# cortes-ciriano-lab/DeMethify

Hardware: AMD Instinct MI355X
Metric: NMF update iters/sec (1e6 CpG x 256 samples x 16 types) (higher is better)
Workload: dtype f64; 1 GPU; headline_1e6x256_12+4; N_cpg=1000000, S_samples=256, n_known=12, n_unknown=4, inner_iters=20, restarts=64, restart_seed=1 + k, restart_placement=k mod n_gpus, parallelism=restart-sharded x1

## Files before the change

### demethify_amd/csrc/dmf_api.h

```cpp
#pragma once
#include <hip/hip_runtime.h>

#include <cmath>
#include <cstdio>
#include <cstdlib>
#include <cstring>
#include <memory>
#include <mutex>
#include <new>
#include <unordered_map>
#include <utility>
#include <vector>

#include "../../include/demethify_hip.h"
#include "dmf_internal.h"
#include "dmf_select.h"

using dmf::SolverState;

namespace dmf_api {

int hip_fail(hipError_t e, const char* what, const char* file, int line);

#define HIP_TRY(expr)                                                                          \
// ... 146 lines not shown
    int64_t N16 = 0, plane_stride = 0;
    dmf_api::DevBuf<unsigned short> X16;
    double x16_dev = 0.0, x16_sum = 0.0;
    bool d_f32_exact = false;
    dmf_api::DevBuf<double> gb_known;
    dmf::GramRan known_ran;
    dmf_api::DevBuf<unsigned char> mask_bits;
    dmf_api::DevBuf<unsigned short> W16;
    int64_t n_test = 0;
    dmf::ProblemView view() const {
        dmf::ProblemView v;
        v.V = V, v.D = D, v.D16 = D16, v.X16 = X16, v.Dt8 = Dt8;
        v.plane_stride = plane_stride, v.SD = SD, v.ND = ND;
        v.Rt = Rt, v.Rtp = Rtp;
        v.N = N, v.S = (int)S, v.n_c = (int)n_c;
        return v;
    }
};

constexpr size_t kPinnedStateBytes = (sizeof(SolverState) + 15) / 16 * 16 + 16;

struct dmf_solver {
    dmf_context* ctx = nullptr;
    const dmf_problem* p = nullptr;
    int64_t n_u = 0;
    int mode = 0;
    dmf::ShapeKey key;
    dmf::PathSpec spec;
    dmf_api::DevBuf<double> cm;
    dmf_api::DevBuf<double> beta_tab;
    int64_t beta_cap = 0;
    dmf_api::DevBuf<long long> slab_i8;
    int64_t slab_i8_words = 0;
    dmf_api::DevBuf<long long> acc_i8;
    dmf_api::DevBuf<double> purity;
    dmf_api::DevBuf<double> u2_partials;
    dmf_api::DevBuf<double> u, u_prev, u_next;
    dmf_api::DevBuf<double> alpha, alpha_prev;
    dmf_api::DevBuf<double> gb;
    dmf::GramRan last_gram;
    int last_gram_source = -1;
    dmf_api::DevBuf<double> slab;
    int64_t slab_doubles = 0;
    dmf_api::DevBuf<double> partials;
    dmf_api::DevBuf<SolverState> state;
    SolverState* h_state = nullptr;
    dmf_api::JobTable jobs;
    bool cf_pending = true;
    double* mom_host = nullptr;
    dmf_api::DevBuf<double> mom_dev;
    hipEvent_t cost_event = nullptr;
    bool cost_pending = false;
    bool in_flight = false;
    bool confirm_stops = false;
    double cf_stream = 0.0;
    long long cf_stream_iter = -1;
    long long n_rowpass = 0, n_rowpass_pair = 0;
    long long n_confirmed = 0, n_unconfirmed = 0;
    dmf::IterateView iterate() const {
        dmf::IterateView it;
        it.u = u, it.u_prev = u_prev, it.alpha = alpha, it.state = state;
        it.n_u = (int)n_u, it.mode = mode;
        return it;
    }
    dmf::AlphaView alpha_view() const {
        dmf::AlphaView a;
        a.gb = gb, a.alpha = alpha, a.alpha_prev = alpha_prev, a.purity = purity, a.state = state, a.partials = partials;
// ... 78 lines not shown
```

### demethify_amd/csrc/dmf_api_problem.hip

```cpp
#include "dmf_api.h"

namespace dmf_api {

static int alloc_count_copies(dmf_problem* p, int ND, bool x16, bool w16) {
    dmf_context* ctx = p->ctx;
    p->ND = ND;
    p->SD = (int)((p->S + 63) / 64 * 64);
    p->N16 = (p->N + 15) / 16 * 16;
    p->plane_stride = ((p->N + 31) / 32) * (p->SD / 32) * 1024;
    const size_t u16_elems = (size_t)p->N16 * p->SD;
    HIP_TRY(p->D16.alloc(ctx, u16_elems));
    HIP_TRY(p->Dt8.alloc(ctx, (size_t)p->plane_stride * ND));
    if (x16) HIP_TRY(p->X16.alloc(ctx, u16_elems));
    if (w16) HIP_TRY(p->W16.alloc(ctx, u16_elems));
    return DMF_OK;
}

static void known_route(dmf_problem* p, const char* piece) {
    char* t = p->known_ran.text;
    const size_t have = std::strlen(t), cap = sizeof(p->known_ran.text);
    snprintf(t + have, cap - have, "%s%s", have > 0 ? " " : "", piece);
}

static int problem_finalize(dmf_problem* p, bool counts_done = false) {
// ... 45 lines not shown
                p->X16.reset();
            } else {
                std::memcpy(&p->x16_dev, &got[1], sizeof(double));
                p->x16_sum = (double)got[2];
            }
        }
    }

    if (n_c > 0 && n_c <= 48) {
        const int nct = (int)((n_c + 3) / 4 * 4);
        if (nct == n_c) {
            p->Rtp.borrow(p->Rt);
        } else {
            HIP_TRY(p->Rtp.alloc(ctx, (size_t)N * nct));
            HIP_TRY(dmf::launch_pad_rows(p->Rt, p->Rtp, N, (int)n_c, nct, ctx->stream));
        }
    }

    const dmf::ProblemView pv = p->view();
    JobTable jobs;
    jobs.build(0, (int)n_c, [](int, int) { return true; });
    const int n_jobs = jobs.n;
    const bool mfma = n_c >= 1 && ctx->generic_level != 1 && ctx->generic_level != 2;
    const int n_fast = mfma ? n_jobs - 1 : 0, n_dense = (int)(n_c * (n_c + 1) / 2);
    const bool int_known = mfma && ctx->generic_level == 0 && p->Dt8 != nullptr && p->D16 != nullptr && p->Rtp != nullptr &&
                           (reinterpret_cast<uintptr_t>(p->Rtp.get()) & 15) == 0 &&
                           dmf::gram_i8_known_supported((int)n_c, p->ND, N, p->SD);
    int64_t slab_doubles = dmf::gram_slab_doubles(N, (int)S, mfma ? 1 : n_jobs);
    if (mfma && !int_known) {
        const int64_t need = dmf::gram_mfma_slab_doubles(N, (int)S, n_fast);
        if (need > slab_doubles) slab_doubles = need;
    }
    DevBuf<double> slab, slab_bu;
    DevBuf<long long> slab_i8, acc;
    HIP_TRY(p->gb_known.alloc(ctx, (size_t)n_jobs * S));
    DMF_TRY(jobs.upload(ctx));
    HIP_TRY(slab.alloc(ctx, (size_t)slab_doubles));
    bool vdv_done = true;
    if (int_known) {
        const int64_t slab_words = dmf::gram_i8_slab_words_nf(N, p->SD, n_dense);
        const int64_t acc_words = dmf::gram_i8_acc_words_nf((int)S, n_dense, (int)n_c + 1);
        HIP_TRY(slab_i8.alloc(ctx, (size_t)slab_words));
        HIP_TRY(acc.alloc(ctx, (size_t)acc_words));
        HIP_TRY(slab_bu.alloc(ctx, (size_t)dmf::bu_cols_grid(N) * (n_c + 1) * S));
        HIP_TRY(hipMemsetAsync(acc, 0, (size_t)acc_words * sizeof(long long), ctx->stream));
        int ny = 0, n_slabs = 0;
        dmf::GramRan ran;
        HIP_TRY(dmf::launch_gram_i8(pv, nullptr, 0, jobs.k, jobs.l, n_dense, slab_i8, slab_words, nullptr, &ny, ctx->stream, &ran));
        known_route(p, "int_known");
        known_route(p, ran.text);
        HIP_TRY(dmf::launch_bu_cols(pv, p->Rt, (int)n_c, slab_bu, nullptr, &n_slabs, ctx->stream, &vdv_done));
        known_route(p, vdv_done ? "+ k_bu_cols2 with vDv" : "+ k_bu_cols");
        HIP_TRY(dmf::launch_gram_v2_reduce(slab_i8, ny, n_dense, p->SD, slab_bu, n_slabs, (int)n_c + (vdv_done ? 1 : 0), (int)S,
                                           acc, jobs.dst, p->gb_known, nullptr, nullptr, 0, nullptr, ctx->stream));
    } else if (mfma) {
        dmf::GramJobTable fast{jobs.k, jobs.l, jobs.dst, n_fast};
        int ny = 0;
        dmf::GramRan ran;
        HIP_TRY(dmf::launch_gram_mfma(pv, nullptr, 0, fast, n_dense, slab, slab_doubles, nullptr, &ny, ctx->stream, &ran));
        known_route(p, "fp64");
        known_route(p, ran.text);
        HIP_TRY(dmf::launch_gram_reduce(slab, ny, n_fast, (int)S, jobs.dst, p->gb_known, nullptr, ctx->stream));
    }
    if (int_known && vdv_done) {
    } else if (n_jobs - n_fast == 1 && ctx->generic_level != 1 && ctx->generic_level != 2 &&
               (int64_t)dmf::vdv_cols_grid(N) * S <= slab_doubles) {
        HIP_TRY(dmf::launch_vdv_cols(pv, slab, p->gb_known + (int64_t)jobs.h_dst[n_jobs - 1] * S, ctx->stream));
        known_route(p, p->known_ran.text[0] == 0 ? "fp64 k_vdv_cols" : "+ k_vdv_cols");
    } else {
        dmf::GramJobTable rest{jobs.k + n_fast, jobs.l + n_fast, jobs.dst + n_fast, n_jobs - n_fast};
        dmf::GramRan ran;
        if (p->known_ran.text[0] == 0) known_route(p, "fp64");
        else known_route(p, "+");
        HIP_TRY(dmf::launch_gram(pv, nullptr, 0, rest, slab, slab_doubles, p->gb_known, nullptr, ctx->stream, &ran));
        known_route(p, ran.text);
    }
    HIP_TRY(hipStreamSynchronize(ctx->stream));
    return DMF_OK;
}

static dmf::CostPlan cost_plan_of(dmf_context* ctx, const dmf::ProblemView& p, int n_u) {
    return dmf::cost_plan(dmf::cost_key(p, n_u, ctx->generic_level));
}

hipError_t enqueue_cost(dmf_context* ctx, const dmf::ProblemView& p, const double* u, const double* alpha, int n_u,
                        double* scratch, double* out) {
    return dmf::launch_cost_plan(cost_plan_of(ctx, p, n_u), p, u, alpha, n_u, scratch, out, ctx->stream);
// ... 251 lines not shown
```

### demethify_amd/csrc/dmf_api_solver.hip

```cpp
#include "dmf_api.h"

namespace dmf_api {

using dmf::kSplitInnerSteps;

static int ensure_split_scratch(dmf_solver* s, int n_iter2) {
    dmf_context* ctx = s->ctx;
    if (s->cm == nullptr) HIP_TRY(s->cm.alloc(ctx, (size_t)dmf::u_phase_split_cm_doubles(s->p->N, (int)s->n_u)));
    if (s->beta_cap < n_iter2 || s->beta_tab == nullptr) {
        s->beta_cap = n_iter2 > 0 ? n_iter2 : 1;
        HIP_TRY(s->beta_tab.alloc(ctx, (size_t)s->beta_cap));
    }
    return DMF_OK;
}

int enqueue_u_phase(dmf_solver* s, int n_iter2, dmf::RowKind row) {
    dmf_context* ctx = s->ctx;
    const dmf::ProblemView pv = s->p->view();
    FamilyScope scope(ctx, DMF_KERNEL_ROWPASS);
    switch (row) {
        case dmf::RowKind::CmI8InnerRows:
            DMF_TRY(ensure_split_scratch(s, n_iter2));
            HIP_TRY(dmf::launch_u_phase_split_i8(pv, s->iterate(), n_iter2, s->scratch(), ctx->stream));
            return DMF_OK;
        case dmf::RowKind::UPhaseBig:
            HIP_TRY(dmf::launch_u_phase_big(pv, s->iterate(), n_iter2, ctx->stream));
            return DMF_OK;
        case dmf::RowKind::UPhaseMfmaSplit:
            DMF_TRY(ensure_split_scratch(s, n_iter2));
            HIP_TRY(dmf::launch_u_phase_split(pv, s->iterate(), n_iter2, s->scratch(), ctx->stream));
            return DMF_OK;
        case dmf::RowKind::UPhaseMfma:
            HIP_TRY(dmf::launch_u_phase_mfma(pv, s->iterate(), n_iter2, ctx->stream));
            return DMF_OK;
        case dmf::RowKind::UPhaseGram:
            HIP_TRY(dmf::launch_u_phase_gram(pv, s->iterate(), n_iter2, ctx->stream));
            return DMF_OK;
        case dmf::RowKind::UStepDirect:
            for (int t = 0; t < n_iter2; ++t) {
                HIP_TRY(dmf::launch_u_step_direct(pv, s->iterate(), s->u_next, t, ctx->stream));
                std::swap(s->u_prev, s->u);
                std::swap(s->u, s->u_next);
            }
            return DMF_OK;
        default: return DMF_ERR_BAD_ARG;
    }
}

dmf::RowKind standalone_row_kind(const dmf_solver* s, int n_iter2) {
    return dmf::plan_iteration(s->key, dmf::standalone_spec(s->spec), n_iter2, false).row;
}

struct GramI8Buffers {
    double* slab_bu = nullptr;
    long long* slab_i8 = nullptr;
    int64_t slab_i8_words = 0;
    long long* acc = nullptr;
    double* gb = nullptr;
    const int* done = nullptr;
};

static GramI8Buffers solver_i8_buffers(dmf_solver* s) {
    GramI8Buffers b;
    b.slab_bu = s->slab, b.slab_i8 = s->slab_i8, b.slab_i8_words = s->slab_i8_words, b.acc = s->acc_i8, b.gb = s->gb;
    b.done = &s->state->done;
    return b;
}

static int gram_i8_and_reduce(dmf_solver* s, const GramI8Buffers& b, int n_slabs, const double* u2_partials, int n_u2,
                              dmf::GramRan* ran = nullptr) {
    dmf_context* ctx = s->ctx;
    const dmf_problem* p = s->p;
    const int S = (int)p->S, n_c = (int)p->n_c, n_u = (int)s->n_u, nf = n_c * n_u + n_u * (n_u + 1) / 2;
    int ny = 0;
    HIP_TRY(dmf::launch_gram_i8(p->view(), s->u, n_u, s->jobs.k, s->jobs.l, nf, b.slab_i8, b.slab_i8_words, b.done, &ny,
                                ctx->stream, ran));
    HIP_TRY(dmf::launch_gram_v2_reduce(b.slab_i8, ny, nf, p->SD, b.slab_bu, n_slabs, n_u, S, b.acc, s->jobs.dst, b.gb, b.done,
                                       u2_partials, n_u2, s->state, ctx->stream));
    return DMF_OK;
}

static int gram_bu_cols_i8(dmf_solver* s, const GramI8Buffers& b, dmf::GramRan* ran = nullptr) {
    int n_slabs = 0;
    HIP_TRY(dmf::launch_bu_cols(s->p->view(), s->u, (int)s->n_u, b.slab_bu, b.done, &n_slabs, s->ctx->stream));
    return gram_i8_and_reduce(s, b, n_slabs, nullptr, 0, ran);
}

int enqueue_gram(dmf_solver* s, dmf::GramKind kind, bool heed_done, dmf::GramRan* ran) {
    dmf_context* ctx = s->ctx;
    const dmf::ProblemView pv = s->p->view();
    const int S = pv.S, n_u = (int)s->n_u;
    const int* done = heed_done ? &s->state->done : nullptr;
    FamilyScope scope(ctx, DMF_KERNEL_GRAM);
    if (kind == dmf::GramKind::BuColsI8) {
        GramI8Buffers b = solver_i8_buffers(s);
        b.done = done;
        return gram_bu_cols_i8(s, b, ran);
    }
    if (kind == dmf::GramKind::GramU) {
        int ny = 0;
        HIP_TRY(dmf::launch_gram_u(pv, s->u, n_u, s->slab, done, &ny, ctx->stream, ran));
        HIP_TRY(dmf::launch_gram_reduce(s->slab, ny, s->jobs.n, S, s->jobs.dst, s->gb, done, ctx->stream));
        return DMF_OK;
    }
    dmf::GramJobTable jobs{s->jobs.k, s->jobs.l, s->jobs.dst, s->jobs.n};
    if (kind == dmf::GramKind::GramMfma) {
        int ny = 0;
        HIP_TRY(dmf::launch_gram_mfma(pv, s->u, n_u, jobs, s->jobs.n - n_u, s->slab, s->slab_doubles, done, &ny, ctx->stream, ran));
        HIP_TRY(dmf::launch_gram_reduce(s->slab, ny, s->jobs.n, S, s->jobs.dst, s->gb, done, ctx->stream));
        return DMF_OK;
    }
// ... 222 lines not shown
    if (s->spec.use_fused) {
        const int64_t spec = dmf::rowpass_fused_slab_doubles(N - (N & 15), (int)S, (int)n_c, (int)n_u) +
                             dmf::gram_u_slab_doubles(16, (int)S, (int)n_c, (int)n_u);
        if (spec > s->slab_doubles) s->slab_doubles = spec;
    }
    if (s->spec.use_v2) {
        const int64_t bu = (int64_t)dmf::rowpass_v2_grid(N, (int)S) * n_u * S;
        if (bu > s->slab_doubles) s->slab_doubles = bu;
    }
    if (s->spec.use_gram_i8) {
        const int64_t bu = (int64_t)dmf::bu_cols_grid(N) * n_u * S;
        if (bu > s->slab_doubles) s->slab_doubles = bu;
        if (s->spec.use_cm_i8) {
            const int64_t bu2 = (int64_t)dmf::u_inner_bu_grid(N, (int)S) * n_u * S;
            if (bu2 > s->slab_doubles) s->slab_doubles = bu2;
        }
    }
    const size_t un = (size_t)N * n_u, an = (size_t)K * S;
    const size_t un_alloc = (un + 1) & ~(size_t)1;
    const size_t gbn = (size_t)(K + 1) * (K + 2) / 2 * S;
    const int nb_alpha = (int)((S + 63) / 64);
    HIP_TRY(s->u.alloc(ctx, un_alloc));
    HIP_TRY(s->u_prev.alloc(ctx, un_alloc));
    if (s->spec.u_path == 2) HIP_TRY(s->u_next.alloc(ctx, un_alloc));
    HIP_TRY(s->alpha.alloc(ctx, an));
    HIP_TRY(s->alpha_prev.alloc(ctx, an));
    HIP_TRY(s->gb.alloc(ctx, gbn));
    HIP_TRY(s->slab.alloc(ctx, (size_t)s->slab_doubles));
    HIP_TRY(s->partials.alloc(ctx, (size_t)2 * (nb_alpha + S)));
    HIP_TRY(s->u2_partials.alloc(ctx, 4096));
    if (s->spec.use_v2 || s->spec.use_gram_i8) {
        s->slab_i8_words = dmf::gram_i8_slab_words(N, p->SD, (int)n_c, (int)n_u);
        HIP_TRY(s->slab_i8.alloc(ctx, (size_t)s->slab_i8_words));
        const size_t acc_words = (size_t)dmf::gram_i8_acc_words((int)S, (int)n_c, (int)n_u);
        HIP_TRY(s->acc_i8.alloc(ctx, acc_words));
        HIP_TRY(hipMemsetAsync(s->acc_i8, 0, acc_words * sizeof(long long), ctx->stream));
    }
    HIP_TRY(s->state.alloc(ctx, 1));
    if (!ctx->pinned_states.empty()) {
        s->h_state = (SolverState*)ctx->pinned_states.back();
        ctx->pinned_states.pop_back();
    } else {
        HIP_TRY(hipHostMalloc((void**)&s->h_state, kPinnedStateBytes));
    }
    const hipMemcpyKind in_kind = (flags & DMF_PTR_DEVICE) ? hipMemcpyDeviceToDevice : hipMemcpyHostToDevice;
    HIP_TRY(hipMemsetAsync(s->state, 0, sizeof(SolverState), ctx->stream));
    HIP_TRY(hipMemsetAsync(s->gb, 0, gbn * sizeof(double), ctx->stream));
    HIP_TRY(hipMemcpyAsync(s->u, u0, un * sizeof(double), in_kind, ctx->stream));
    HIP_TRY(hipMemcpyAsync(s->u_prev, s->u, un * sizeof(double), hipMemcpyDeviceToDevice, ctx->stream));
    HIP_TRY(hipMemcpyAsync(s->alpha, alpha0, an * sizeof(double), in_kind, ctx->stream));
    HIP_TRY(hipMemcpyAsync(s->alpha_prev, s->alpha, an * sizeof(double), hipMemcpyDeviceToDevice, ctx->stream));
    DMF_TRY(s->jobs.upload(ctx));
    HIP_TRY(dmf::launch_scatter_known_block(p->gb_known, s->gb, (int)n_c, (int)K, (int)S, ctx->stream));
    HIP_TRY(dmf::launch_sumsq_f64(s->u, N * n_u, ctx->scratch, &s->state->u_norm2, nullptr, ctx->stream));
    HIP_TRY(dmf::launch_init_state(s->state, p->consts, s->alpha, (int)S, (int)n_c, (int)n_u, ctx->stream));
    if (!(flags & DMF_PTR_DEVICE)) HIP_TRY(hipStreamSynchronize(ctx->stream));
    return DMF_OK;
}

}

using namespace dmf_api;

extern "C" {

int dmf_solver_create(dmf_context* ctx, const dmf_problem* p, const double* u0, const double* alpha0,
                      int64_t n_u, int mode, int flags, dmf_solver** out) {
    DMF_TRY(check_ctx(ctx));
    if (out == nullptr) return DMF_ERR_BAD_ARG;
// ... 140 lines not shown
    *out_cost = *cost_slot(s);
    return DMF_OK;
}

int dmf_solver_holdout_error(dmf_solver* s, const dmf_problem* full, double* sum_sq, int64_t* n_test) {
    if (s == nullptr || full == nullptr || sum_sq == nullptr || n_test == nullptr) return DMF_ERR_BAD_ARG;
    dmf_context* ctx = s->ctx;
    DMF_TRY(check_ctx(ctx));
    const dmf_problem* p = s->p;
    if (p->mask_bits == nullptr || full->mask_bits != nullptr || full->ctx != ctx) return DMF_ERR_BAD_ARG;
    if (full->N != p->N || full->S != p->S || full->n_c != p->n_c) return DMF_ERR_BAD_SHAPE;
    *n_test = p->n_test;
    *sum_sq = 0.0;
    if (p->n_test == 0) return DMF_OK;
    dmf::ProblemView pv;
    pv.N = p->N, pv.S = (int)p->S, pv.n_c = (int)p->n_c;
    pv.V = full->V, pv.Rt = p->Rt, pv.Rtp = p->Rtp;
    pv.D16 = p->W16, pv.SD = p->SD;
    DevBuf<double> weights;
    if (!cost_reads_u16_only(ctx, pv, (int)s->n_u)) {
        HIP_TRY(weights.alloc(ctx, (size_t)p->N * p->S));
        HIP_TRY(dmf::launch_holdout_weights_f64(p->mask_bits, weights, p->N, (int)p->S, ctx->stream));
        pv.D = weights, pv.D16 = nullptr, pv.SD = 0;
    }
    return cost_to_host(ctx, pv, s->u, s->alpha, (int)s->n_u, sum_sq, true);
}

static int solver_gram_enqueue(dmf_solver* s, int kind, double* out_gb, dmf::GramRan* ran) {
    dmf_context* ctx = s->ctx;
    const dmf_problem* p = s->p;
    const int64_t N = p->N, S = p->S, n_c = p->n_c, n_u = s->n_u, K = n_c + n_u;
    const size_t gbn = (size_t)(K + 1) * (K + 2) / 2 * S;
    DevBuf<double> slab_bu;
    DevBuf<long long> slab_i8, acc;
    if (kind == DMF_GRAM_LAST) {
        *ran = s->last_gram;
    } else if (kind == DMF_GRAM_FP64) {
        DMF_TRY(enqueue_gram(s, fp64_gram_kind(s), false, ran));
    } else {
        GramI8Buffers b;
        b.slab_i8_words = dmf::gram_i8_slab_words(N, p->SD, (int)n_c, (int)n_u);
        const size_t acc_words = (size_t)dmf::gram_i8_acc_words((int)S, (int)n_c, (int)n_u);
        HIP_TRY(slab_bu.alloc(ctx, (size_t)dmf::bu_cols_grid(N) * n_u * S));
        HIP_TRY(slab_i8.alloc(ctx, (size_t)b.slab_i8_words));
        HIP_TRY(acc.alloc(ctx, acc_words));
        HIP_TRY(hipMemsetAsync(acc, 0, acc_words * sizeof(long long), ctx->stream));
        b.slab_bu = slab_bu, b.slab_i8 = slab_i8, b.acc = acc, b.gb = s->gb;
        FamilyScope scope(ctx, DMF_KERNEL_GRAM);
        DMF_TRY(gram_bu_cols_i8(s, b, ran));
    }
    HIP_TRY(hipMemcpyAsync(out_gb, s->gb, gbn * sizeof(double), hipMemcpyDeviceToHost, ctx->stream));
    HIP_TRY(hipStreamSynchronize(ctx->stream));
    return DMF_OK;
}

int dmf_solver_gram(dmf_solver* s, int kind, double* out_gb, char* out_text, int64_t cap) {
    if (s == nullptr || out_gb == nullptr || (kind != DMF_GRAM_INTEGER && kind != DMF_GRAM_FP64 && kind != DMF_GRAM_LAST))
        return DMF_ERR_BAD_ARG;
    if (out_text != nullptr && cap < 1) return DMF_ERR_BAD_ARG;
    dmf_context* ctx = s->ctx;
    DMF_TRY(check_ctx(ctx));
    const dmf_problem* p = s->p;
    if (kind == DMF_GRAM_INTEGER &&
        (p->ND < 1 || p->D16 == nullptr || p->Dt8 == nullptr || (p->n_c > 0 && p->Rtp == nullptr) ||
         (reinterpret_cast<uintptr_t>(p->Rtp.get()) & 15) != 0 ||
         !dmf::gram_i8_supported((int)p->n_c, (int)s->n_u, p->ND, p->N, p->SD)))
        return DMF_ERR_UNSUPPORTED;
    dmf::GramRan ran;
    s->in_flight = true;
    const int status = solver_gram_enqueue(s, kind, out_gb, &ran);
    if (status != DMF_OK) (void)hipStreamSynchronize(ctx->stream);
    s->in_flight = false;
    if (status == DMF_OK && out_text != nullptr) snprintf(out_text, (size_t)cap, "%s", ran.text);
    return status;
}

static dmf::RowKind row_moments_kind(const dmf_solver* s) { return standalone_row_kind(s, kSplitInnerSteps + 1); }

static int solver_row_moments_enqueue(dmf_solver* s, dmf::RowKind row, double* out_cm, dmf::CmRan* ran) {
    dmf_context* ctx = s->ctx;
// ... 114 lines not shown
```

### demethify_amd/csrc/dmf_internal.h

```cpp
#pragma once
#include <hip/hip_runtime.h>
#include <stdint.h>

#include "dmf_select.h"

namespace dmf {

struct SolverState {
    double a1;
    double a2;
    double l_w;
    double l_w_prev;
    double l_h;
    double l_h_prev;
    double dsq;
    double rt_norm2;
    double u_norm2;
    double cf;
    double cf_prev;
    double tol;
    long long iters;
    double band;
    int done;
    int arrive;
// ... 246 lines not shown
constexpr double kX16MaxDev = 8.0 * 0x1p-53;
hipError_t launch_build_counts_int(const double* D, const double* V, int64_t N, int S, int ND, unsigned short* D16,
                                   unsigned short* X16, int64_t N16, int SD, signed char* Dt8, int64_t plane_stride,
                                   unsigned long long* x_stats, hipStream_t st);
hipError_t launch_build_dt8(const unsigned short* D16, int64_t N, int SD, int ND, signed char* Dt8, int64_t plane_stride,
                            hipStream_t st);
hipError_t launch_mask_problem(const double* srcV, const double* srcD, const unsigned short* src16,
                               const unsigned short* srcX, const unsigned char* bits, double* dstV, double* dstD,
                               unsigned short* dst16, unsigned short* dstX, unsigned short* W16, int64_t N, int64_t N16, int S,
                               int SD, unsigned long long* stats, hipStream_t st);
hipError_t launch_holdout_weights_f64(const unsigned char* bits, double* W, int64_t N, int S, hipStream_t st);
constexpr int64_t kMaskDrawMaxS = ((int64_t)1 << 31) - 1, kMaskDrawMaxElements = (int64_t)1 << 60;
hipError_t launch_mask_draw(unsigned int* key_io, int pos, int64_t N, int64_t S, unsigned long long threshold,
                            unsigned char* bits, unsigned long long* result, hipStream_t st);
bool rowpass_v2_supported(int S, int n_c, int n_u, int n_iter2);
int rowpass_v2_grid(int64_t N, int S);
hipError_t launch_rowpass_v2(const ProblemView& p, const IterateView& it, int n_iter2, const UScratch& scratch, int* grid_out,
                             bool pair, bool* paired_out, hipStream_t st);
bool rowpass_v2_pair_fits(int S, int n_u, int n_iter2);
bool gram_i8_supported(int n_c, int n_u, int ND, int64_t N, int SD);
struct GramI8Plan {
    bool supported = false;
    int xl = 1, nd = 1, ring = 8;
    int nf = 0, launches = 0;
    int nsh = 0, ny = 0;
    int64_t rows_per_wg = 0;
    int blocks = 0, last = 0;
    int tail = 0;
    bool xcd = false;
};
GramI8Plan gram_i8_plan(int64_t N, int SD, int n_c, int n_u, int ND);
void describe_gram_i8_plan(const GramI8Plan& g, char* buf, size_t cap);
int64_t gram_i8_slab_words(int64_t N, int SD, int n_c, int n_u);
int64_t gram_i8_acc_words(int S, int n_c, int n_u);
bool gram_i8_known_supported(int n_c, int ND, int64_t N, int SD);
int64_t gram_i8_slab_words_nf(int64_t N, int SD, int nf);
int64_t gram_i8_acc_words_nf(int S, int nf, int n_bu);
hipError_t launch_gram_i8(const ProblemView& p, const double* u, int n_u, const short* feat_a, const short* feat_b, int NF,
                          long long* slab, int64_t slab_words, const int* done_flag, int* ny_out, hipStream_t st,
                          GramRan* ran = nullptr);
int bu_cols_grid(int64_t N);
hipError_t launch_bu_cols(const ProblemView& p, const double* u, int n_u, double* slab, const int* done_flag,
                          int* n_slabs_out, hipStream_t st, bool* with_vdv = nullptr);
hipError_t launch_gram_v2_reduce(const long long* slab_i8, int ny, int NF, int SD, const double* slab_bu, int n_bu_slabs,
                                 int n_u, int S, long long* acc_words, const int* dst_row, double* gb, const int* done_flag,
                                 const double* u2_partials, int n_u2, SolverState* state, hipStream_t st);

hipError_t launch_percentile_pair(const double* x, int64_t n, int64_t m, PercentilePlan p0, PercentilePlan p1,
                                  double* out0, double* out1, hipStream_t st);
hipError_t launch_nanpercentile_pair(const double* x, int64_t n, int64_t m, PercentilePlan p0, PercentilePlan p1, double q0,
                                     double q1, double* out0, double* out1, hipStream_t st);
int64_t percentile_max_replicates();

int wls_moments_grid(int64_t N);
int64_t wls_slab_doubles(int64_t N, int S, int K);
hipError_t launch_wls_moments(const ProblemView& p, const double* u, int n_u, int target_dv, double* slab, double* mom,
                              hipStream_t st);
hipError_t launch_nnls_intercept(const double* gb, const double* mom, int K, int S, double* out, int* status, hipStream_t st);

constexpr int kSvdMaxS = 512, kSvdMaxNc = 64, kSvdMaxRank = 64;
constexpr size_t kSvdMaxLds = 160 * 1024;
size_t svd_project_lds_bytes(int S, int rank);
struct SvdColumns {
    double sign[kSvdMaxRank], scale[kSvdMaxRank];
};
bool svd_supported(int S, int n_c, int rank);
int svd_gram_grid(int64_t N, int S);
int64_t svd_gram_slab_doubles(int64_t N, int S);
hipError_t launch_svd_gram(const ProblemView& p, const double* H1, double* slab, int* flags, double* C, hipStream_t st);
int64_t svd_project_slab_doubles(int64_t N, int rank);
hipError_t launch_svd_project(const ProblemView& p, const double* H1, const double* Es, int rank, double* T, double* slab,
                              double* norms, hipStream_t st);
hipError_t launch_svd_finish(double* T, int64_t N, int rank, const SvdColumns& cols, hipStream_t st);

struct MatchColumns {
    int src[kMaxK];
};
int match_gram_grid(int64_t N, int n_u);
// ... 13 lines not shown
```

### demethify_amd/csrc/dmf_kernels_gram_i8.hip

```cpp
#include <cstdint>
#include <cstdio>
#include <cstdlib>

#include "dmf_device.h"
#include "dmf_dispatch.h"
#include "dmf_internal.h"
#include "dmf_fixedpoint.h"

namespace dmf {

typedef int v4i __attribute__((ext_vector_type(4)));
typedef int v16i __attribute__((ext_vector_type(16)));
typedef unsigned int v4u __attribute__((ext_vector_type(4)));

namespace {
constexpr int kNSL = 7;
constexpr int kRing = 8;
constexpr int kMaxFeat = 576;
}

__global__ __launch_bounds__(256) void k_build_d16(const double* __restrict__ D, const double* __restrict__ V, int64_t N, int S,
                                                   unsigned short* __restrict__ D16, unsigned short* __restrict__ X16,
                                                   int64_t N16, int SD, unsigned long long* __restrict__ x_stats) {
    const int64_t chunks = N16 * (SD / 8);
// ... 588 lines not shown
    }
}

int bu_cols_grid(int64_t N) {
    int64_t want = (N + 4 * 8 - 1) / (4 * 8);
    if (want > 512) want = 512;
    return (int)(want < 1 ? 1 : want);
}

hipError_t launch_bu_cols(const ProblemView& p, const double* u, int n_u, double* slab, const int* done_flag,
                          int* n_slabs_out, hipStream_t st, bool* with_vdv) {
    const int S = p.S, nbx = bu_cols_grid(p.N);
    *n_slabs_out = nbx;
    const dim3 block(256);
    const bool two = (p.SD & 1) == 0 && S >= 128 && n_u <= 16 && (p.v_align() & 7) == 0;
    const int vdv = (with_vdv != nullptr && *with_vdv && two) ? 1 : 0;
    if (with_vdv != nullptr) *with_vdv = vdv != 0;
    if (two && n_u >= 1) {
        const dim3 grid2(nbx, (S + 127) / 128);
        return dispatch_int<1, 16>(n_u, [&](auto nu) {
            hipLaunchKernelGGL((k_bu_cols2<decltype(nu)::value>), grid2, block, 0, st, p.V, p.D16, p.SD, u, p.N, S, slab,
                               done_flag, vdv);
            return hipGetLastError();
        });
    }
    const dim3 grid(nbx, (S + 63) / 64);
    return dispatch_int<1, 32>(n_u, [&](auto nu) {
        hipLaunchKernelGGL((k_bu_cols<decltype(nu)::value>), grid, block, 0, st, p.V, p.D16, p.SD, u, p.N, S, slab, done_flag);
        return hipGetLastError();
    });
}

constexpr int kRedChunks = 16;

__global__ __launch_bounds__(256) void k_gram_v2_reduce(const long long* __restrict__ slab_i8, int ny, int MF, int SDs,
                                                        const double* __restrict__ slab_bu, int n_bu_slabs, int n_u,
                                                        int n_feat, int S, unsigned long long* __restrict__ acc64,
                                                        double* __restrict__ bu_part,
                                                        const int* __restrict__ done_flag,
                                                        const double* __restrict__ u2_partials, int n_u2,
                                                        SolverState* __restrict__ state) {
    __shared__ long long part[3][2][64];
    __shared__ double partd[3][64];
    if (done_flag != nullptr && *done_flag) return;
    const int lane = threadIdx.x & 63, grp = threadIdx.x >> 6;
    const int s = blockIdx.x * 64 + lane;
    const int job = blockIdx.y, chunk = blockIdx.z;
    const bool active = s < S;
    const int sc = active ? s : S - 1;
    if (u2_partials != nullptr && blockIdx.x == 0 && job == 0 && chunk == 0 && grp == 3) {
        double a = 0.0;
        for (int i = lane; i < n_u2; i += 64) a += u2_partials[i];
        a = wave_sum(a);
        if (lane == 0) {
            state->u_norm2 = a;
            state->l_h = (state->rt_norm2 + a) * state->dsq;
        }
    }
    if (job < n_feat) {
        const int per = (ny + kRedChunks - 1) / kRedChunks;
        const int y0 = chunk * per, y1 = y0 + per < ny ? y0 + per : ny;
        const int64_t hi_off = (int64_t)MF * SDs, y_stride = (int64_t)2 * MF * SDs;
        const long long* __restrict__ base = slab_i8 + (int64_t)job * SDs + sc;
        long long lo = 0, hi = 0;
        for (int y = y0 + grp; y < y1; y += 16) {
            long long l[4], h[4];
#pragma unroll
            for (int q = 0; q < 4; ++q) {
                const int yy = y + 4 * q;
                const long long* __restrict__ b = base + (int64_t)(yy < y1 ? yy : y) * y_stride;
                l[q] = b[0];
                h[q] = b[hi_off];
            }
#pragma unroll
            for (int q = 0; q < 4; ++q)
                if (y + 4 * q < y1) {
                    lo += l[q];
                    hi += h[q];
                }
        }
        if (grp > 0) {
            part[grp - 1][0][lane] = lo;
            part[grp - 1][1][lane] = hi;
        }
        __syncthreads();
        if (grp == 0 && active && y0 < y1) {
            lo += part[0][0][lane] + part[1][0][lane] + part[2][0][lane];
            hi += part[0][1][lane] + part[1][1][lane] + part[2][1][lane];
            atomicAdd(acc64 + (int64_t)job * S + s, (unsigned long long)lo);
            atomicAdd(acc64 + ((int64_t)n_feat + job) * S + s, (unsigned long long)hi);
        }
    } else {
        const int j = job - n_feat;
        const int per = (n_bu_slabs + kRedChunks - 1) / kRedChunks;
        const int c0 = chunk * per, c1 = c0 + per < n_bu_slabs ? c0 + per : n_bu_slabs;
        const int perw = (per + 3) / 4;
        const int g0 = c0 + grp * perw, g1 = g0 + perw < c1 ? g0 + perw : c1;
        const double* __restrict__ base = slab_bu + (int64_t)j * S + sc;
        const int64_t g_stride = (int64_t)n_u * S;
        double acc = 0.0;
        for (int g = g0; g < g1; g += 4) {
            double v[4];
#pragma unroll
            for (int q = 0; q < 4; ++q) v[q] = base[(int64_t)(g + q < g1 ? g + q : g) * g_stride];
#pragma unroll
            for (int q = 0; q < 4; ++q)
                if (g + q < g1) acc += v[q];
        }
        if (grp > 0) partd[grp - 1][lane] = acc;
        __syncthreads();
        if (grp == 0 && active) bu_part[((int64_t)chunk * n_u + j) * S + s] = ((acc + partd[0][lane]) + partd[1][lane]) + partd[2][lane];
    }
}

__global__ __launch_bounds__(64) void k_gram_v2_finish(int n_u, int n_feat, int S, unsigned long long* __restrict__ acc64,
                                                       double* __restrict__ bu_part, const int* __restrict__ dst_row,
                                                       double* __restrict__ gb, const int* __restrict__ done_flag) {
    if (done_flag != nullptr && *done_flag) return;
    const int s = blockIdx.x * 64 + threadIdx.x;
    const int job = blockIdx.y;
    if (s >= S) return;
    if (job < n_feat) {
        unsigned long long* __restrict__ plo = acc64 + (int64_t)job * S + s;
        unsigned long long* __restrict__ phi = acc64 + ((int64_t)n_feat + job) * S + s;
        const long long lo = (long long)*plo, hi = (long long)*phi;
        *plo = 0ull;
        *phi = 0ull;
        gb[(int64_t)dst_row[job] * S + s] = fma((double)hi, 0x1p32, (double)lo) * 0x1p-52;
    } else {
        const int j = job - n_feat;
        double acc = 0.0;
        for (int c = 0; c < kRedChunks; ++c) acc += bu_part[((int64_t)c * n_u + j) * S + s];
        gb[(int64_t)dst_row[job] * S + s] = acc;
    }
}

void gram_i8_geometry(int64_t N, int SD, int* nsh, int* ny, int64_t* rows_per_wg) {
    const int SB = SD / 32;
    *nsh = (SB + 3) / 4;
    int want = 256 / *nsh;
    if (want < 1) want = 1;
    int64_t rpw = ((N + want - 1) / want + 31) / 32 * 32;
    if (rpw < 32) rpw = 32;
    *rows_per_wg = rpw;
    *ny = (int)((N + rpw - 1) / rpw);
}

GramI8Plan gram_i8_plan(int64_t N, int SD, int n_c, int n_u, int ND) {
    GramI8Plan g;
    if (N < 1 || SD < 64 || SD % 64 != 0 || n_c < 0 || n_u < 0) return g;
    const int nct = (n_c + 3) / 4 * 4;
    g.nf = n_u > 0 ? n_c * n_u + n_u * (n_u + 1) / 2 : n_c * (n_c + 1) / 2;
    g.nd = ND;
    g.xl = nct + n_u > 16 ? 2 : 1;
    g.ring = g.xl == 2 && ND == 2 ? 6 : kRing;
    g.launches = (g.nf + 63) / 64;
    gram_i8_geometry(N, SD, &g.nsh, &g.ny, &g.rows_per_wg);
    g.blocks = (int)(g.rows_per_wg / 32);
    g.last = (int)((N - (int64_t)(g.ny - 1) * g.rows_per_wg + 31) / 32);
    g.tail = (int)(N & 31);
    g.xcd = g.ny % 8 == 0;
    g.supported = nct + n_u <= 32 && g.nf >= 1 && g.nf <= kMaxFeat && ND >= 1 && ND <= 2 &&
                  g.rows_per_wg * 128 * 128 * ND < (int64_t)1 << 31;
    return g;
}

void describe_gram_i8_plan(const GramI8Plan& g, char* buf, size_t cap) {
    snprintf(buf, cap, "k_gram_i8_w8<%d,%d,%d> launches=%d nsh=%d ny=%d blocks=%d last=%d tail=%d xcd=%d", g.xl, g.nd, g.ring,
             g.launches, g.nsh, g.ny, g.blocks, g.last, g.tail, g.xcd ? 1 : 0);
}

bool gram_i8_supported(int n_c, int n_u, int ND, int64_t N, int SD) {
    return n_u >= 1 && gram_i8_plan(N, SD, n_c, n_u, ND).supported;
}

bool gram_i8_known_supported(int n_c, int ND, int64_t N, int SD) { return gram_i8_plan(N, SD, n_c, 0, ND).supported; }
int64_t gram_i8_slab_words_nf(int64_t N, int SD, int nf) {
    int nsh, ny;
    int64_t rpw;
    gram_i8_geometry(N, SD, &nsh, &ny, &rpw);
    return (int64_t)ny * 2 * ((nf + 31) / 32 * 32) * SD;
}
int64_t gram_i8_acc_words_nf(int S, int nf, int n_bu) { return (int64_t)2 * nf * S + (int64_t)kRedChunks * n_bu * S; }

int64_t gram_i8_slab_words(int64_t N, int SD, int n_c, int n_u) {
    const int nf = n_c * n_u + n_u * (n_u + 1) / 2;
    int nsh, ny;
    int64_t rpw;
    gram_i8_geometry(N, SD, &nsh, &ny, &rpw);
    return (int64_t)ny * 2 * ((nf + 31) / 32 * 32) * SD;
}
int64_t gram_i8_acc_words(int S, int n_c, int n_u) {
    const int nf = n_c * n_u + n_u * (n_u + 1) / 2;
    return (int64_t)2 * nf * S + (int64_t)kRedChunks * n_u * S;
}

size_t gram_i8_w8_lds_bytes(int xl, int nd, int ring) { return (size_t)ring * (4096 * nd + xl * 4096) + (size_t)3 * 2 * (kNSL * 64) * 16; }

hipError_t launch_gram_i8(const ProblemView& p, const double* u, int n_u, const short* fa, const short* fb, int NF,
                          long long* slab, int64_t slab_words, const int* done_flag, int* ny_out, hipStream_t st, GramRan* ran) {
    const int SD = p.SD, n_c = p.n_c;
    const GramI8Plan g = gram_i8_plan(p.N, SD, n_c, n_u, p.ND);
    if (!g.supported || g.nf != NF) return hipErrorInvalidValue;
    const int ny = g.ny;
    *ny_out = ny;
    const int MFtot = (NF + 31) / 32 * 32;
    if ((int64_t)ny * 2 * MFtot * SD > slab_words) return hipErrorInvalidValue;
    const int chunk = 64;
    int launches = 0;
    for (int p0 = 0; p0 < NF; p0 += chunk) {
        const int nf = NF - p0 < chunk ? NF - p0 : chunk;
        const hipError_t e = dispatch_bool(g.nd == 1, [&](auto one_digit) {
            return dispatch_bool(g.xl == 2, [&](auto wide_t) {
                constexpr int XL = decltype(wide_t)::value ? 2 : 1, ND = decltype(one_digit)::value ? 1 : 2;
                constexpr int RING = XL == 2 && ND == 2 ? 6 : kRing;
                if (RING != g.ring) return hipErrorInvalidValue;
                const size_t lds = gram_i8_w8_lds_bytes(XL, ND, RING);
                const hipError_t e_lds = raise_dynamic_lds<k_gram_i8_w8<XL, ND, RING>>(lds);
                if (e_lds != hipSuccess) return e_lds;
                hipLaunchKernelGGL((k_gram_i8_w8<XL, ND, RING>), dim3(g.nsh * ny), dim3(512), lds, st, p.Dt8, p.plane_stride, SD / 32,
                                   p.Rtp, (n_c + 3) / 4 * 4, u, p.N, n_c, n_u, fa, fb, nf, p0, MFtot, g.rows_per_wg, slab, SD,
                                   done_flag
#ifdef DMF_STAMPS
                                   , (unsigned long long*)nullptr
#endif
                                   );
                return hipGetLastError();
            });
        });
        if (e != hipSuccess) return e;
        ++launches;
    }
    if (launches != g.launches) return hipErrorInvalidValue;
    if (ran != nullptr) describe_gram_i8_plan(g, ran->text, sizeof(ran->text));
    return hipSuccess;
}

hipError_t launch_gram_v2_reduce(const long long* slab_i8, int ny, int NF, int SD, const double* slab_bu, int n_bu_slabs,
                                 int n_u, int S, long long* acc_words, const int* dst_row, double* gb, const int* done_flag,
                                 const double* u2_partials, int n_u2, SolverState* state, hipStream_t st) {
    const int MF = (NF + 31) / 32 * 32;
    unsigned long long* acc64 = reinterpret_cast<unsigned long long*>(acc_words);
    double* bu_part = reinterpret_cast<double*>(acc_words + (int64_t)2 * NF * S);
    hipLaunchKernelGGL(k_gram_v2_reduce, dim3((S + 63) / 64, NF + n_u, kRedChunks), dim3(256), 0, st, slab_i8, ny, MF, SD,
                       slab_bu, n_bu_slabs, n_u, NF, S, acc64, bu_part, done_flag, u2_partials, n_u2, state);
    hipLaunchKernelGGL(k_gram_v2_finish, dim3((S + 63) / 64, NF + n_u), dim3(64), 0, st, n_u, NF, S, acc64, bu_part, dst_row,
                       gb, done_flag);
    return hipGetLastError();
}

}
```

Before: 1797 outer iters/s.

## Fuse gram v2 reduce and finish into one single-pass sum kernel without atomics

Replaces the two-kernel reduction (chunked partial sums with 64-bit atomics into an accumulator, then a finish kernel that converts and clears it) with one kernel. Each block of 16 waves sums all y-slabs for its job and sample tile, then reduces across waves in shared memory and writes gb directly. The b_u part is split four ways per sample tile to keep enough blocks. This removes one launch, the atomic traffic, the accumulator buffer and its memset, at the cost of fewer, larger blocks that each do a longer serial loop.

```diff
diff --git a/demethify_amd/csrc/dmf_api.h b/demethify_amd/csrc/dmf_api.h
--- a/demethify_amd/csrc/dmf_api.h
+++ b/demethify_amd/csrc/dmf_api.h
@@ -202,7 +202,6 @@
     int64_t beta_cap = 0;
     dmf_api::DevBuf<long long> slab_i8;
     int64_t slab_i8_words = 0;
-    dmf_api::DevBuf<long long> acc_i8;
     dmf_api::DevBuf<double> purity;
     dmf_api::DevBuf<double> u2_partials;
     dmf_api::DevBuf<double> u, u_prev, u_next;
diff --git a/demethify_amd/csrc/dmf_api_problem.hip b/demethify_amd/csrc/dmf_api_problem.hip
--- a/demethify_amd/csrc/dmf_api_problem.hip
+++ b/demethify_amd/csrc/dmf_api_problem.hip
@@ -101,18 +101,15 @@
         if (need > slab_doubles) slab_doubles = need;
     }
     DevBuf<double> slab, slab_bu;
-    DevBuf<long long> slab_i8, acc;
+    DevBuf<long long> slab_i8;
     HIP_TRY(p->gb_known.alloc(ctx, (size_t)n_jobs * S));
     DMF_TRY(jobs.upload(ctx));
     HIP_TRY(slab.alloc(ctx, (size_t)slab_doubles));
     bool vdv_done = true;
     if (int_known) {
         const int64_t slab_words = dmf::gram_i8_slab_words_nf(N, p->SD, n_dense);
-        const int64_t acc_words = dmf::gram_i8_acc_words_nf((int)S, n_dense, (int)n_c + 1);
         HIP_TRY(slab_i8.alloc(ctx, (size_t)slab_words));
-        HIP_TRY(acc.alloc(ctx, (size_t)acc_words));
         HIP_TRY(slab_bu.alloc(ctx, (size_t)dmf::bu_cols_grid(N) * (n_c + 1) * S));
-        HIP_TRY(hipMemsetAsync(acc, 0, (size_t)acc_words * sizeof(long long), ctx->stream));
         int ny = 0, n_slabs = 0;
         dmf::GramRan ran;
         HIP_TRY(dmf::launch_gram_i8(pv, nullptr, 0, jobs.k, jobs.l, n_dense, slab_i8, slab_words, nullptr, &ny, ctx->stream, &ran));
@@ -121,7 +118,7 @@
         HIP_TRY(dmf::launch_bu_cols(pv, p->Rt, (int)n_c, slab_bu, nullptr, &n_slabs, ctx->stream, &vdv_done));
         known_route(p, vdv_done ? "+ k_bu_cols2 with vDv" : "+ k_bu_cols");
         HIP_TRY(dmf::launch_gram_v2_reduce(slab_i8, ny, n_dense, p->SD, slab_bu, n_slabs, (int)n_c + (vdv_done ? 1 : 0), (int)S,
-                                           acc, jobs.dst, p->gb_known, nullptr, nullptr, 0, nullptr, ctx->stream));
+                                           jobs.dst, p->gb_known, nullptr, nullptr, 0, nullptr, ctx->stream));
     } else if (mfma) {
         dmf::GramJobTable fast{jobs.k, jobs.l, jobs.dst, n_fast};
         int ny = 0;
diff --git a/demethify_amd/csrc/dmf_api_solver.hip b/demethify_amd/csrc/dmf_api_solver.hip
--- a/demethify_amd/csrc/dmf_api_solver.hip
+++ b/demethify_amd/csrc/dmf_api_solver.hip
@@ -55,14 +55,13 @@
     double* slab_bu = nullptr;
     long long* slab_i8 = nullptr;
     int64_t slab_i8_words = 0;
-    long long* acc = nullptr;
     double* gb = nullptr;
     const int* done = nullptr;
 };
 
 static GramI8Buffers solver_i8_buffers(dmf_solver* s) {
     GramI8Buffers b;
-    b.slab_bu = s->slab, b.slab_i8 = s->slab_i8, b.slab_i8_words = s->slab_i8_words, b.acc = s->acc_i8, b.gb = s->gb;
+    b.slab_bu = s->slab, b.slab_i8 = s->slab_i8, b.slab_i8_words = s->slab_i8_words, b.gb = s->gb;
     b.done = &s->state->done;
     return b;
 }
@@ -75,8 +74,8 @@
     int ny = 0;
     HIP_TRY(dmf::launch_gram_i8(p->view(), s->u, n_u, s->jobs.k, s->jobs.l, nf, b.slab_i8, b.slab_i8_words, b.done, &ny,
                                 ctx->stream, ran));
-    HIP_TRY(dmf::launch_gram_v2_reduce(b.slab_i8, ny, nf, p->SD, b.slab_bu, n_slabs, n_u, S, b.acc, s->jobs.dst, b.gb, b.done,
-                                       u2_partials, n_u2, s->state, ctx->stream));
+    HIP_TRY(dmf::launch_gram_v2_reduce(b.slab_i8, ny, nf, p->SD, b.slab_bu, n_slabs, n_u, S, s->jobs.dst, b.gb, b.done, u2_partials,
+                                       n_u2, s->state, ctx->stream));
     return DMF_OK;
 }
 
@@ -365,9 +364,6 @@
     if (s->spec.use_v2 || s->spec.use_gram_i8) {
         s->slab_i8_words = dmf::gram_i8_slab_words(N, p->SD, (int)n_c, (int)n_u);
         HIP_TRY(s->slab_i8.alloc(ctx, (size_t)s->slab_i8_words));
-        const size_t acc_words = (size_t)dmf::gram_i8_acc_words((int)S, (int)n_c, (int)n_u);
-        HIP_TRY(s->acc_i8.alloc(ctx, acc_words));
-        HIP_TRY(hipMemsetAsync(s->acc_i8, 0, acc_words * sizeof(long long), ctx->stream));
     }
     HIP_TRY(s->state.alloc(ctx, 1));
     if (!ctx->pinned_states.empty()) {
@@ -574,7 +570,7 @@
     const int64_t N = p->N, S = p->S, n_c = p->n_c, n_u = s->n_u, K = n_c + n_u;
     const size_t gbn = (size_t)(K + 1) * (K + 2) / 2 * S;
     DevBuf<double> slab_bu;
-    DevBuf<long long> slab_i8, acc;
+    DevBuf<long long> slab_i8;
     if (kind == DMF_GRAM_LAST) {
         *ran = s->last_gram;
     } else if (kind == DMF_GRAM_FP64) {
@@ -582,12 +578,9 @@
     } else {
         GramI8Buffers b;
         b.slab_i8_words = dmf::gram_i8_slab_words(N, p->SD, (int)n_c, (int)n_u);
-        const size_t acc_words = (size_t)dmf::gram_i8_acc_words((int)S, (int)n_c, (int)n_u);
         HIP_TRY(slab_bu.alloc(ctx, (size_t)dmf::bu_cols_grid(N) * n_u * S));
         HIP_TRY(slab_i8.alloc(ctx, (size_t)b.slab_i8_words));
-        HIP_TRY(acc.alloc(ctx, acc_words));
-        HIP_TRY(hipMemsetAsync(acc, 0, acc_words * sizeof(long long), ctx->stream));
-        b.slab_bu = slab_bu, b.slab_i8 = slab_i8, b.acc = acc, b.gb = s->gb;
+        b.slab_bu = slab_bu, b.slab_i8 = slab_i8, b.gb = s->gb;
         FamilyScope scope(ctx, DMF_KERNEL_GRAM);
         DMF_TRY(gram_bu_cols_i8(s, b, ran));
     }
diff --git a/demethify_amd/csrc/dmf_internal.h b/demethify_amd/csrc/dmf_internal.h
--- a/demethify_amd/csrc/dmf_internal.h
+++ b/demethify_amd/csrc/dmf_internal.h
@@ -302,10 +302,8 @@
 GramI8Plan gram_i8_plan(int64_t N, int SD, int n_c, int n_u, int ND);
 void describe_gram_i8_plan(const GramI8Plan& g, char* buf, size_t cap);
 int64_t gram_i8_slab_words(int64_t N, int SD, int n_c, int n_u);
-int64_t gram_i8_acc_words(int S, int n_c, int n_u);
 bool gram_i8_known_supported(int n_c, int ND, int64_t N, int SD);
 int64_t gram_i8_slab_words_nf(int64_t N, int SD, int nf);
-int64_t gram_i8_acc_words_nf(int S, int nf, int n_bu);
 hipError_t launch_gram_i8(const ProblemView& p, const double* u, int n_u, const short* feat_a, const short* feat_b, int NF,
                           long long* slab, int64_t slab_words, const int* done_flag, int* ny_out, hipStream_t st,
                           GramRan* ran = nullptr);
@@ -313,7 +311,7 @@
 hipError_t launch_bu_cols(const ProblemView& p, const double* u, int n_u, double* slab, const int* done_flag,
                           int* n_slabs_out, hipStream_t st, bool* with_vdv = nullptr);
 hipError_t launch_gram_v2_reduce(const long long* slab_i8, int ny, int NF, int SD, const double* slab_bu, int n_bu_slabs,
-                                 int n_u, int S, long long* acc_words, const int* dst_row, double* gb, const int* done_flag,
+                                 int n_u, int S, const int* dst_row, double* gb, const int* done_flag,
                                  const double* u2_partials, int n_u2, SolverState* state, hipStream_t st);
 
 hipError_t launch_percentile_pair(const double* x, int64_t n, int64_t m, PercentilePlan p0, PercentilePlan p1,
diff --git a/demethify_amd/csrc/dmf_kernels_gram_i8.hip b/demethify_amd/csrc/dmf_kernels_gram_i8.hip
--- a/demethify_amd/csrc/dmf_kernels_gram_i8.hip
+++ b/demethify_amd/csrc/dmf_kernels_gram_i8.hip
@@ -644,106 +644,109 @@
 }
 
 constexpr int kRedChunks = 16;
-
-__global__ __launch_bounds__(256) void k_gram_v2_reduce(const long long* __restrict__ slab_i8, int ny, int MF, int SDs,
-                                                        const double* __restrict__ slab_bu, int n_bu_slabs, int n_u,
-                                                        int n_feat, int S, unsigned long long* __restrict__ acc64,
-                                                        double* __restrict__ bu_part,
-                                                        const int* __restrict__ done_flag,
-                                                        const double* __restrict__ u2_partials, int n_u2,
-                                                        SolverState* __restrict__ state) {
-    __shared__ long long part[3][2][64];
-    __shared__ double partd[3][64];
+constexpr int kSumWaves = 16;
+constexpr int kSumBatch = 8;
+constexpr int kSumBuBatch = 16;
+constexpr int kSumBuSplit = 4;
+static_assert(kSumWaves == kRedChunks, "a wave of a b_u job sums one chunk");
+
+__global__ __launch_bounds__(64 * kSumWaves, 8) void k_gram_v2_sum(const long long* __restrict__ slab_i8, int ny, int MF, int SDs,
+                                                                   const double* __restrict__ slab_bu, int n_bu_slabs, int n_u,
+                                                                   int n_feat, int S, const int* __restrict__ dst_row,
+                                                                   double* __restrict__ gb, const int* __restrict__ done_flag,
+                                                                   const double* __restrict__ u2_partials, int n_u2,
+                                                                   SolverState* __restrict__ state) {
+    __shared__ long long part[kSumWaves - 1][2][64];
+    __shared__ double piece_sum[kRedChunks][4][64 / kSumBuSplit];
     if (done_flag != nullptr && *done_flag) return;
-    const int lane = threadIdx.x & 63, grp = threadIdx.x >> 6;
-    const int s = blockIdx.x * 64 + lane;
-    const int job = blockIdx.y, chunk = blockIdx.z;
-    const bool active = s < S;
-    const int sc = active ? s : S - 1;
-    if (u2_partials != nullptr && blockIdx.x == 0 && job == 0 && chunk == 0 && grp == 3) {
+    const int lane = threadIdx.x & 63, wave = __builtin_amdgcn_readfirstlane(threadIdx.x >> 6);
+    if (blockIdx.y < n_feat) {
+        const int job = blockIdx.y;
+        const int64_t row = dst_row[job];
+        const int s = blockIdx.x * 64 + lane;
+        const bool active = s < S;
+        const int sc = active ? s : S - 1;
+        const int64_t hi_off = (int64_t)MF * SDs, y_stride = (int64_t)2 * MF * SDs;
+        const long long* __restrict__ base = slab_i8 + (int64_t)job * SDs + sc;
+        long long lo = 0, hi = 0;
+        for (int y = wave; y < ny; y += kSumWaves * kSumBatch) {
+            long long l[kSumBatch], h[kSumBatch];
+#pragma unroll
+            for (int q = 0; q < kSumBatch; ++q) {
+                const int yy = y + kSumWaves * q;
+                const long long* __restrict__ b = base + (int64_t)(yy < ny ? yy : y) * y_stride;
+                l[q] = b[0];
+                h[q] = b[hi_off];
+            }
+#pragma unroll
+            for (int q = 0; q < kSumBatch; ++q)
+                if (y + kSumWaves * q < ny) {
+                    lo += l[q];
+                    hi += h[q];
+                }
+        }
+        if (wave > 0) {
+            part[wave - 1][0][lane] = lo;
+            part[wave - 1][1][lane] = hi;
+        }
+        __syncthreads();
+        if (wave == 0 && active) {
+#pragma unroll
+            for (int w = 0; w < kSumWaves - 1; ++w) {
+                lo += part[w][0][lane];
+                hi += part[w][1][lane];
+            }
+            gb[row * S + s] = fma((double)hi, 0x1p32, (double)lo) * 0x1p-52;
+        }
+    } else {
+        constexpr int kSamples = 64 / kSumBuSplit;
+        const int yb = blockIdx.y - n_feat, j = yb / kSumBuSplit;
+        const int s0 = blockIdx.x * 64 + (yb % kSumBuSplit) * kSamples;
+        if (s0 >= S) return;
+        const int64_t row = dst_row[n_feat + j];
+        const int q = lane / kSamples, sl = lane % kSamples, s = s0 + sl;
+        const bool active = s < S;
+        const int sc = active ? s : S - 1;
+        const int per = (n_bu_slabs + kRedChunks - 1) / kRedChunks, perw = (per + 3) / 4;
+        const int c1 = (wave + 1) * per < n_bu_slabs ? (wave + 1) * per : n_bu_slabs;
+        const int g0 = wave * per + q * perw, g1 = g0 + perw < c1 ? g0 + perw : c1;
+        const double* __restrict__ base = slab_bu + (int64_t)j * S + sc;
+        const int64_t g_stride = (int64_t)n_u * S;
+        double p = 0.0;
+        for (int t = 0; t < perw; t += kSumBuBatch) {
+            double v[kSumBuBatch];
+#pragma unroll
+            for (int e = 0; e < kSumBuBatch; ++e)
+                v[e] = base[(int64_t)(g0 + t + e < g1 ? g0 + t + e : 0) * g_stride];
+#pragma unroll
+            for (int e = 0; e < kSumBuBatch; ++e)
+                if (g0 + t + e < g1) p += v[e];
+        }
+        piece_sum[wave][q][sl] = p;
+        __syncthreads();
+        if (wave == 0 && lane < kSamples && active) {
+            double acc = 0.0;
+#pragma unroll
+            for (int c = 0; c < kRedChunks; ++c)
+                acc += ((piece_sum[c][0][lane] + piece_sum[c][1][lane]) + piece_sum[c][2][lane]) + piece_sum[c][3][lane];
+            gb[row * S + s] = acc;
+        }
+    }
+    if (u2_partials != nullptr && blockIdx.x == 0 && blockIdx.y == 0 && wave == kSumWaves - 1) {
         double a = 0.0;
-        for (int i = lane; i < n_u2; i += 64) a += u2_partials[i];
+        for (int i = lane; i < n_u2; i += 64 * 8) {
+            double v[8];
+#pragma unroll
+            for (int e = 0; e < 8; ++e) v[e] = u2_partials[i + 64 * e < n_u2 ? i + 64 * e : i];
+#pragma unroll
+            for (int e = 0; e < 8; ++e)
+                if (i + 64 * e < n_u2) a += v[e];
+        }
         a = wave_sum(a);
         if (lane == 0) {
             state->u_norm2 = a;
             state->l_h = (state->rt_norm2 + a) * state->dsq;
         }
-    }
-    if (job < n_feat) {
-        const int per = (ny + kRedChunks - 1) / kRedChunks;
-        const int y0 = chunk * per, y1 = y0 + per < ny ? y0 + per : ny;
-        const int64_t hi_off = (int64_t)MF * SDs, y_stride = (int64_t)2 * MF * SDs;
-        const long long* __restrict__ base = slab_i8 + (int64_t)job * SDs + sc;
-        long long lo = 0, hi = 0;
-        for (int y = y0 + grp; y < y1; y += 16) {
-            long long l[4], h[4];
-#pragma unroll
-            for (int q = 0; q < 4; ++q) {
-                const int yy = y + 4 * q;
-                const long long* __restrict__ b = base + (int64_t)(yy < y1 ? yy : y) * y_stride;
-                l[q] = b[0];
-                h[q] = b[hi_off];
-            }
-#pragma unroll
-            for (int q = 0; q < 4; ++q)
-                if (y + 4 * q < y1) {
-                    lo += l[q];
-                    hi += h[q];
-                }
-        }
-        if (grp > 0) {
-            part[grp - 1][0][lane] = lo;
-            part[grp - 1][1][lane] = hi;
-        }
-        __syncthreads();
-        if (grp == 0 && active && y0 < y1) {
-            lo += part[0][0][lane] + part[1][0][lane] + part[2][0][lane];
-            hi += part[0][1][lane] + part[1][1][lane] + part[2][1][lane];
-            atomicAdd(acc64 + (int64_t)job * S + s, (unsigned long long)lo);
-            atomicAdd(acc64 + ((int64_t)n_feat + job) * S + s, (unsigned long long)hi);
-        }
-    } else {
-        const int j = job - n_feat;
-        const int per = (n_bu_slabs + kRedChunks - 1) / kRedChunks;
-        const int c0 = chunk * per, c1 = c0 + per < n_bu_slabs ? c0 + per : n_bu_slabs;
-        const int perw = (per + 3) / 4;
-        const int g0 = c0 + grp * perw, g1 = g0 + perw < c1 ? g0 + perw : c1;
-        const double* __restrict__ base = slab_bu + (int64_t)j * S + sc;
-        const int64_t g_stride = (int64_t)n_u * S;
-        double acc = 0.0;
-        for (int g = g0; g < g1; g += 4) {
-            double v[4];
-#pragma unroll
-            for (int q = 0; q < 4; ++q) v[q] = base[(int64_t)(g + q < g1 ? g + q : g) * g_stride];
-#pragma unroll
-            for (int q = 0; q < 4; ++q)
-                if (g + q < g1) acc += v[q];
-        }
-        if (grp > 0) partd[grp - 1][lane] = acc;
-        __syncthreads();
-        if (grp == 0 && active) bu_part[((int64_t)chunk * n_u + j) * S + s] = ((acc + partd[0][lane]) + partd[1][lane]) + partd[2][lane];
-    }
-}
-
-__global__ __launch_bounds__(64) void k_gram_v2_finish(int n_u, int n_feat, int S, unsigned long long* __restrict__ acc64,
-                                                       double* __restrict__ bu_part, const int* __restrict__ dst_row,
-                                                       double* __restrict__ gb, const int* __restrict__ done_flag) {
-    if (done_flag != nullptr && *done_flag) return;
-    const int s = blockIdx.x * 64 + threadIdx.x;
-    const int job = blockIdx.y;
-    if (s >= S) return;
-    if (job < n_feat) {
-        unsigned long long* __restrict__ plo = acc64 + (int64_t)job * S + s;
-        unsigned long long* __restrict__ phi = acc64 + ((int64_t)n_feat + job) * S + s;
-        const long long lo = (long long)*plo, hi = (long long)*phi;
-        *plo = 0ull;
-        *phi = 0ull;
-        gb[(int64_t)dst_row[job] * S + s] = fma((double)hi, 0x1p32, (double)lo) * 0x1p-52;
-    } else {
-        const int j = job - n_feat;
-        double acc = 0.0;
-        for (int c = 0; c < kRedChunks; ++c) acc += bu_part[((int64_t)c * n_u + j) * S + s];
-        gb[(int64_t)dst_row[job] * S + s] = acc;
     }
 }
 
@@ -793,7 +796,6 @@
     gram_i8_geometry(N, SD, &nsh, &ny, &rpw);
     return (int64_t)ny * 2 * ((nf + 31) / 32 * 32) * SD;
 }
-int64_t gram_i8_acc_words_nf(int S, int nf, int n_bu) { return (int64_t)2 * nf * S + (int64_t)kRedChunks * n_bu * S; }
 
 int64_t gram_i8_slab_words(int64_t N, int SD, int n_c, int n_u) {
     const int nf = n_c * n_u + n_u * (n_u + 1) / 2;
@@ -801,10 +803,6 @@
     int64_t rpw;
     gram_i8_geometry(N, SD, &nsh, &ny, &rpw);
     return (int64_t)ny * 2 * ((nf + 31) / 32 * 32) * SD;
-}
-int64_t gram_i8_acc_words(int S, int n_c, int n_u) {
-    const int nf = n_c * n_u + n_u * (n_u + 1) / 2;
-    return (int64_t)2 * nf * S + (int64_t)kRedChunks * n_u * S;
 }
 
 size_t gram_i8_w8_lds_bytes(int xl, int nd, int ring) { return (size_t)ring * (4096 * nd + xl * 4096) + (size_t)3 * 2 * (kNSL * 64) * 16; }
@@ -849,15 +847,11 @@
 }
 
 hipError_t launch_gram_v2_reduce(const long long* slab_i8, int ny, int NF, int SD, const double* slab_bu, int n_bu_slabs,
-                                 int n_u, int S, long long* acc_words, const int* dst_row, double* gb, const int* done_flag,
+                                 int n_u, int S, const int* dst_row, double* gb, const int* done_flag,
                                  const double* u2_partials, int n_u2, SolverState* state, hipStream_t st) {
     const int MF = (NF + 31) / 32 * 32;
-    unsigned long long* acc64 = reinterpret_cast<unsigned long long*>(acc_words);
-    double* bu_part = reinterpret_cast<double*>(acc_words + (int64_t)2 * NF * S);
-    hipLaunchKernelGGL(k_gram_v2_reduce, dim3((S + 63) / 64, NF + n_u, kRedChunks), dim3(256), 0, st, slab_i8, ny, MF, SD,
-                       slab_bu, n_bu_slabs, n_u, NF, S, acc64, bu_part, done_flag, u2_partials, n_u2, state);
-    hipLaunchKernelGGL(k_gram_v2_finish, dim3((S + 63) / 64, NF + n_u), dim3(64), 0, st, n_u, NF, S, acc64, bu_part, dst_row,
-                       gb, done_flag);
+    hipLaunchKernelGGL(k_gram_v2_sum, dim3((S + 63) / 64, NF + kSumBuSplit * n_u), dim3(64 * kSumWaves), 0, st, slab_i8, ny, MF, SD,
+                       slab_bu, n_bu_slabs, n_u, NF, S, dst_row, gb, done_flag, u2_partials, n_u2, state);
     return hipGetLastError();
 }
 
```

After: 1807 outer iters/s, median of 6. About the same (+0.5%).
